# mkkellogg/GaussianSplats3D

Measured on NVIDIA H100. Metric: frames_per_sec, higher is better.
Workload: dtype int32 sort keys / f32 raster

## Files before the change

### gaussiansplats3d_b200/csrc/common.cuh

```cuda
#pragma once
#include <cuda_runtime.h>
#include <stdint.h>
#include <stdio.h>

extern thread_local char g_gs_err[512];

#include <vector>
#include <string.h>
#include <stdlib.h>

namespace gs {

__device__ __forceinline__ void pdl_enter() {
    asm volatile("griddepcontrol.launch_dependents;" ::: "memory");
    asm volatile("griddepcontrol.wait;" ::: "memory");
}
inline bool pdl_enabled() {
    static int on = -1;
    if (on < 0) { const char *v = getenv("GS_PDL"); on = (v && v[0] == '0') ? 0 : 1; }
    return on != 0;
}
template <typename... KArgs, typename... Args>
static inline void gs_launch(void (*kernel)(KArgs...), dim3 grid, dim3 block, size_t smem, cudaStream_t st, Args... args) {
    cudaLaunchConfig_t cfg{};
    cfg.gridDim = grid; cfg.blockDim = block; cfg.dynamicSmemBytes = smem; cfg.stream = st;
    cudaLaunchAttribute attr[1];
    attr[0].id = cudaLaunchAttributeProgrammaticStreamSerialization;
    attr[0].val.programmaticStreamSerializationAllowed = pdl_enabled() ? 1 : 0;
    cfg.attrs = attr; cfg.numAttrs = 1;
    (void)cudaLaunchKernelEx(&cfg, kernel, KArgs(args)...);
}

struct Profiler {
    bool on = false;
    std::vector<cudaEvent_t> ev;
    std::vector<const char *> names;
    size_t used = 0;
    void begin(cudaStream_t st) { used = 0; names.clear(); mark("<begin>", st); }
    void mark(const char *name, cudaStream_t st) {
        if (!on) return;
        if (used == ev.size()) { cudaEvent_t e; cudaEventCreate(&e); ev.push_back(e); }
        cudaEventRecord(ev[used++], st);
        names.push_back(name);
    }
    void release() { for (auto e : ev) cudaEventDestroy(e); ev.clear(); used = 0; }
};

#define GS_MAX_SCENES_DEV 32

constexpr int kRadixBits = 8;
constexpr int kRadix = 1 << kRadixBits;

__device__ __forceinline__ int4 ld_nc_v4(const void *p) {
    int4 r;
    asm volatile("ld.global.nc.L1::no_allocate.v4.s32 {%0,%1,%2,%3}, [%4];" : "=r"(r.x), "=r"(r.y), "=r"(r.z), "=r"(r.w) : "l"(p));
    return r;
}
__device__ __forceinline__ uint32_t ld_nc_u32(const void *p) {
    uint32_t r;
    asm volatile("ld.global.nc.L1::no_allocate.u32 %0, [%1];" : "=r"(r) : "l"(p));
    return r;
}
__device__ __forceinline__ uint32_t ld_volatile_u32(const uint32_t *p) {
    uint32_t r;
    asm volatile("ld.volatile.global.u32 %0, [%1];" : "=r"(r) : "l"(p) : "memory");
    return r;
}
__device__ __forceinline__ uint32_t ld_acquire_u32(const uint32_t *p) {
    uint32_t r;
    asm volatile("ld.acquire.gpu.global.u32 %0, [%1];" : "=r"(r) : "l"(p) : "memory");
    return r;
}
__device__ __forceinline__ void st_release_u32(uint32_t *p, uint32_t v) {
    asm volatile("st.release.gpu.global.u32 [%0], %1;" ::"l"(p), "r"(v) : "memory");
}
__device__ __forceinline__ uint32_t lanemask_lt() {
    uint32_t m;
    asm("mov.u32 %0, %%lanemask_lt;" : "=r"(m));
    return m;
}
__device__ __forceinline__ int warp_min(int v) {
#pragma unroll
    for (int o = 16; o > 0; o >>= 1) v = min(v, __shfl_xor_sync(0xffffffffu, v, o));
    return v;
}
__device__ __forceinline__ int warp_max(int v) {
#pragma unroll
    for (int o = 16; o > 0; o >>= 1) v = max(v, __shfl_xor_sync(0xffffffffu, v, o));
    return v;
}
__device__ __forceinline__ uint32_t warp_inclusive_scan(uint32_t v) {
    const int lane = threadIdx.x & 31;
#pragma unroll
    for (int o = 1; o < 32; o <<= 1) {
        uint32_t t = __shfl_up_sync(0xffffffffu, v, o);
        if (lane >= o) v += t;
    }
    return v;
}

template <int THREADS>
__device__ __forceinline__ uint32_t block_exclusive_scan(uint32_t v, uint32_t *smem_warp , uint32_t &total) {
    const int lane = threadIdx.x & 31, warp = threadIdx.x >> 5;
    constexpr int NW = THREADS / 32;
    const uint32_t inc = warp_inclusive_scan(v);
    if (lane == 31) smem_warp[warp] = inc;
    __syncthreads();
    if (warp == 0) {
        uint32_t w = lane < NW ? smem_warp[lane] : 0u;
        uint32_t wi = warp_inclusive_scan(w);
        smem_warp[lane] = wi - w;
        if (lane == 31) smem_warp[32] = wi;
    }
// ... 18 lines not shown
```

### gaussiansplats3d_b200/csrc/engine.cu

```cuda
#include "../../include/gsplat_b200.h"
#include "common.cuh"
#include "sort_kernels.cuh"
#include "raster_kernels.cuh"
#include "shard_kernels.cuh"
#include "ksplat_transform.h"
#include "ksplat_kernels.cuh"
#include "file_kernels.cuh"
#include "cull_kernels.cuh"

#include <algorithm>
#include <cmath>
#include <cstdarg>
#include <cstdlib>
#include <cstring>
#include <new>
#include <vector>

using namespace gs;

thread_local char g_gs_err[512] = "";
#define g_err g_gs_err
static int fail(int code, const char *fmt, ...) {
    va_list ap;
    va_start(ap, fmt);
    vsnprintf(g_err, sizeof(g_err), fmt, ap);
    va_end(ap);
    return code;
}
#define CU(call)                                                                                                  \
    do {                                                                                                          \
        cudaError_t _e = (call);                                                                                  \
        if (_e != cudaSuccess) return fail(GS_ERR_CUDA, "%s -> %s (%s:%d)", #call, cudaGetErrorString(_e), __FILE__, __LINE__); \
    } while (0)

extern "C" int gs_abi_version(void) { return GS_ABI_VERSION; }
extern "C" const char *gs_last_error_message(void) { return g_err; }
extern "C" const char *gs_status_string(int s) {
    switch (s) {
        case GS_OK: return "ok";
        case GS_ERR_BAD_ARG: return "bad argument";
        case GS_ERR_NO_DEVICE: return "no CUDA device";
        case GS_ERR_CUDA: return "CUDA error";
        case GS_ERR_DEGENERATE: return "all distances equal";
        case GS_ERR_BUCKET_RANGE: return "bucket index out of range";
        case GS_ERR_NOT_READY: return "not ready";
        case GS_ERR_CAPACITY: return "capacity exceeded";
        default: return "unknown";
    }
}
extern "C" int gs_device_count(void) {
    int n = 0;
    if (cudaGetDeviceCount(&n) != cudaSuccess) { cudaGetLastError(); return 0; }
    return n;
}

template <typename T> struct DevBuf {
    T *p = nullptr;
    size_t n = 0;
    int ensure(size_t count) {
        if (count <= n) return GS_OK;
        if (p) cudaFree(p);
        p = nullptr; n = 0;
        cudaError_t e = cudaMalloc((void **)&p, std::max<size_t>(count, 1) * sizeof(T));
        if (e != cudaSuccess) return fail(GS_ERR_CUDA, "cudaMalloc(%zu bytes) -> %s", count * sizeof(T), cudaGetErrorString(e));
        n = count;
        return GS_OK;
    }
    void release() { if (p) cudaFree(p); p = nullptr; n = 0; }
};
template <typename T> struct PinBuf {
    T *p = nullptr;
    size_t n = 0;
    int ensure(size_t count) {
        if (count <= n) return GS_OK;
        if (p) cudaFreeHost(p);
        p = nullptr; n = 0;
        cudaError_t e = cudaHostAlloc((void **)&p, std::max<size_t>(count, 1) * sizeof(T), cudaHostAllocDefault);
        if (e != cudaSuccess) return fail(GS_ERR_CUDA, "cudaHostAlloc(%zu bytes) -> %s", count * sizeof(T), cudaGetErrorString(e));
        n = count;
        return GS_OK;
    }
    void release() { if (p) cudaFreeHost(p); p = nullptr; n = 0; }
};

enum { EV_SORT0, EV_DEPTH, EV_BUCKET, EV_SORT1, EV_R0, EV_PROJECT, EV_BIN, EV_R1, EV_H2D0, EV_H2D1, EV_D2H0, EV_D2H1, EV_COUNT };

constexpr size_t kPipeSlotWords = 4 + (sizeof(RasterControl) + 3) / 4 + 12;
struct gs_engine {
    gs_config cfg{};
    cudaStream_t stream = nullptr;
    cudaEvent_t ev[EV_COUNT]{};
    int sm_count = 132;
    size_t l2_bytes = 50u << 20;
    int key_bits = 16;

    DevBuf<int4> centers;
    DevBuf<uint32_t> scene_idx;
    DevBuf<uint32_t> indexes;
    DevBuf<uint32_t> precomputed;
    DevBuf<int32_t> dist;
    DevBuf<uint32_t> keys[2];
    DevBuf<uint32_t> vals[2];
    DevBuf<uint32_t> sorted;
    DevBuf<float> transforms;
    DevBuf<SortControl> ctl;
    DevBuf<DepthParams> depthp;
    DevBuf<uint32_t> tile_hist;
    DevBuf<uint32_t> freq;
    DevBuf<int32_t> dist_rows_i;
    DevBuf<float> dist_rows_f;
    DevBuf<uint32_t> sub_idx;
    DevBuf<int32_t> sub_dist;
    uint32_t uploaded_splats = 0;
    uint32_t last_render_count = 0;
    bool have_sorted = false;
    bool ctl_dirty = true;

    PinBuf<uint32_t> h_indexes, h_sorted;
    PinBuf<uint32_t> h_ctl;
    PinBuf<unsigned char> h_frame;

    RasterState rs;

    gs_timings tm{};
    Profiler prof;
    cudaGraphExec_t graph_exec = nullptr;
    cudaStream_t stream2 = nullptr;
    cudaEvent_t ev_fork = nullptr, ev_join = nullptr;
    unsigned long long graph_key[8] = {0};
    bool graph_enabled = true;
    bool last_frame_was_graph = false;
    bool no_subset = false;
    uint32_t graph_launches = 0;
    bool have_prof_begin = false;
    bool pending_async = false;
    gs_render_params pending_rp{};
    DevBuf<uint32_t> flush;
    struct Tree {
        DevBuf<double> center, nmin, nmax;
        DevBuf<uint32_t> offsets, indexes, start;
        DevBuf<unsigned long long> key, total;
        uint32_t count = 0, splats = 0;
    } tree;
    cudaStream_t copy_stream = nullptr;
    static constexpr int kPipeRing = 4, kPipeMaxInflight = 3;
    cudaEvent_t ev_frame_done[kPipeRing] = {nullptr}, ev_copy_done[kPipeRing] = {nullptr};
    cudaStream_t param_stream = nullptr;
    cudaEvent_t ev_params[2] = {nullptr, nullptr};
    bool param_side = false;
    bool graph_snapshot[2] = {false, false};
    DevBuf<uint32_t> status_dev;
    cudaGraphExec_t graph_exec_alt = nullptr;
    unsigned long long graph_key_alt[8] = {0};
    PinBuf<uint32_t> h_pipe;
    uint64_t pipe_begun = 0, pipe_ended = 0;
    uint32_t pipe_inflight() const { return (uint32_t)(pipe_begun - pipe_ended); }

    struct Shard {
        DevBuf<unsigned char> block;
        DevBuf<uint32_t> total, ahead, block_total, delta, local_sorted;
        ShardPeers peers{};
        uint32_t *root_out = nullptr;
        void *opened[kMaxShardRanks + 1] = {nullptr};
        uint32_t world = 0, seq = 0;
        uint32_t pending_render_count = 0;
        bool attached = false, pending = false;
        bool pending_unsplit = false;
    } shard;
};

static int check_engine(gs_engine *e) {
    if (!e) return fail(GS_ERR_BAD_ARG, "null engine");
    cudaError_t ce = cudaSetDevice(e->cfg.device);
    if (ce != cudaSuccess) return fail(GS_ERR_CUDA, "cudaSetDevice(%d) -> %s", e->cfg.device, cudaGetErrorString(ce));
    return GS_OK;
}

extern "C" void gs_destroy(gs_engine *e);
#define CUE(call)                                                                                                 \
    do {                                                                                                          \
        cudaError_t _e = (call);                                                                                  \
        if (_e != cudaSuccess) {                                                                                  \
            gs_destroy(e);                                                                                        \
            return fail(GS_ERR_CUDA, "%s -> %s (%s:%d)", #call, cudaGetErrorString(_e), __FILE__, __LINE__);      \
        }                                                                                                         \
    } while (0)
extern "C" int gs_create(const gs_config *cfg, gs_engine **out) {
    if (!cfg || !out) return fail(GS_ERR_BAD_ARG, "gs_create: null argument");
    *out = nullptr;
    gs_config c{};
    memcpy(&c, cfg, std::min<size_t>(cfg->struct_size ? cfg->struct_size : sizeof(gs_config), sizeof(gs_config)));
    if (c.distance_map_range == 0) c.distance_map_range = 1u << 16;
    if (c.distance_map_range < 2 || c.distance_map_range > (1u << 24)) return fail(GS_ERR_BAD_ARG, "distance_map_range %u outside [2, 2^24]", c.distance_map_range);
    if (c.world_size == 0) { c.world_size = 1; c.rank = 0; }
    if (c.rank >= c.world_size) return fail(GS_ERR_BAD_ARG, "rank %u >= world_size %u", c.rank, c.world_size);
    int ndev = gs_device_count();
    if (ndev <= 0) return fail(GS_ERR_NO_DEVICE, "no CUDA device visible: libgsplat_b200 has no CPU path");
    if (c.device < 0 || c.device >= ndev) return fail(GS_ERR_BAD_ARG, "device %d not in [0,%d)", c.device, ndev);
    CU(cudaSetDevice(c.device));
    gs_engine *e = new (std::nothrow) gs_engine();
    if (!e) return fail(GS_ERR_BAD_ARG, "out of host memory");
    e->cfg = c;
    cudaDeviceProp prop{};
    CUE(cudaGetDeviceProperties(&prop, c.device));
    e->sm_count = prop.multiProcessorCount;
    if (prop.l2CacheSize > 0) e->l2_bytes = (size_t)prop.l2CacheSize;
    CUE(cudaStreamCreateWithFlags(&e->stream, cudaStreamNonBlocking));
    CUE(cudaStreamCreateWithFlags(&e->stream2, cudaStreamNonBlocking));
    CUE(cudaEventCreateWithFlags(&e->ev_fork, cudaEventDisableTiming));
    CUE(cudaEventCreateWithFlags(&e->ev_join, cudaEventDisableTiming));
    for (int i = 0; i < EV_COUNT; ++i) CUE(cudaEventCreate(&e->ev[i]));
    int kb = 0;
    while ((1u << kb) < c.distance_map_range) ++kb;
    e->key_bits = kb;
    int rc = GS_OK;
    const size_t n = std::max<uint32_t>(c.max_splat_count, 1);
    if ((rc = e->centers.ensure(n)) || (rc = e->indexes.ensure(n)) || (rc = e->dist.ensure(n)) || (rc = e->sorted.ensure(n)) ||
        (rc = e->vals[0].ensure(n)) || (rc = e->vals[1].ensure(n)) || (rc = e->keys[0].ensure(n)) || (rc = e->keys[1].ensure(n)) ||
        (rc = e->ctl.ensure(1)) || (rc = e->depthp.ensure(2)) || (rc = e->transforms.ensure(16 * GS_MAX_SCENES)) || (rc = e->h_ctl.ensure(sizeof(SortControl) / 4 + 64 + sizeof(RasterControl) / 4 + sizeof(ShardHeader) / 4))) {
        gs_destroy(e);
        return rc;
    }
    if (c.dynamic_mode && (rc = e->scene_idx.ensure(n))) { gs_destroy(e); return rc; }
    if (e->scene_idx.p) CUE(cudaMemsetAsync(e->scene_idx.p, 0, e->scene_idx.n * 4, e->stream));
    {
        std::vector<float> id(16 * GS_MAX_SCENES, 0.f);
        for (int s = 0; s < GS_MAX_SCENES; ++s) id[16 * s] = id[16 * s + 5] = id[16 * s + 10] = id[16 * s + 15] = 1.f;
        CUE(cudaMemcpy(e->transforms.p, id.data(), id.size() * 4, cudaMemcpyHostToDevice));
    }
    CUE(cudaMemset(e->ctl.p, 0, sizeof(SortControl)));
    rc = raster_init(e->rs, c, e->sm_count);
    if (rc) { gs_destroy(e); return fail(rc, "raster_init failed: %s", g_err); }
    if ((rc = e->status_dev.ensure(2 * kPipeSlotWords))) { gs_destroy(e); return rc; }
    CUE(cudaMemset(e->status_dev.p, 0, 2 * kPipeSlotWords * 4));
    e->rs.snap_base = e->status_dev.p;
    e->rs.snap_stride = (uint32_t)kPipeSlotWords;
    e->rs.snap_sort_ctl = reinterpret_cast<const uint32_t *>(e->ctl.p);
    CUE(cudaStreamSynchronize(e->stream));
    *out = e;
    return GS_OK;
}

#undef CUE

extern "C" void gs_destroy(gs_engine *e) {
    if (!e) return;
    cudaSetDevice(e->cfg.device);
    if (e->stream) cudaStreamSynchronize(e->stream);
    e->centers.release(); e->scene_idx.release(); e->indexes.release(); e->precomputed.release(); e->dist.release();
    e->keys[0].release(); e->keys[1].release(); e->vals[0].release(); e->vals[1].release(); e->sorted.release();
    e->transforms.release(); e->ctl.release(); e->depthp.release(); e->tile_hist.release(); e->freq.release(); e->dist_rows_i.release(); e->dist_rows_f.release(); e->sub_idx.release(); e->sub_dist.release();
    e->h_indexes.release(); e->h_sorted.release(); e->h_ctl.release(); e->h_frame.release(); e->h_pipe.release();
    e->tree.center.release(); e->tree.nmin.release(); e->tree.nmax.release(); e->tree.offsets.release(); e->tree.indexes.release(); e->tree.start.release(); e->tree.key.release(); e->tree.total.release(); e->flush.release(); e->prof.release();
    e->shard.block.release(); e->shard.total.release(); e->shard.ahead.release(); e->shard.block_total.release(); e->shard.delta.release(); e->shard.local_sorted.release();
    for (void *m : e->shard.opened) if (m) cudaIpcCloseMemHandle(m);
    if (e->rs.peer_attached) { if (e->rs.peer_frame) cudaIpcCloseMemHandle(e->rs.peer_frame); if (e->rs.peer_sync) cudaIpcCloseMemHandle(e->rs.peer_sync); }
    raster_release(e->rs);
    for (int i = 0; i < EV_COUNT; ++i) if (e->ev[i]) cudaEventDestroy(e->ev[i]);
    if (e->stream) cudaStreamDestroy(e->stream);
    if (e->stream2) cudaStreamDestroy(e->stream2);
    if (e->copy_stream) cudaStreamDestroy(e->copy_stream);
    for (int i = 0; i < gs_engine::kPipeRing; ++i) { if (e->ev_frame_done[i]) cudaEventDestroy(e->ev_frame_done[i]); if (e->ev_copy_done[i]) cudaEventDestroy(e->ev_copy_done[i]); }
    for (int i = 0; i < 2; ++i) if (e->ev_params[i]) cudaEventDestroy(e->ev_params[i]);
    if (e->param_stream) cudaStreamDestroy(e->param_stream);
    e->status_dev.release();
    if (e->graph_exec) cudaGraphExecDestroy(e->graph_exec);
    if (e->graph_exec_alt) cudaGraphExecDestroy(e->graph_exec_alt);
    if (e->ev_fork) cudaEventDestroy(e->ev_fork);
    if (e->ev_join) cudaEventDestroy(e->ev_join);
    delete e;
}

extern "C" int gs_upload_centers(gs_engine *e, const void *centers, const uint32_t *sceneIndexes, uint32_t from, uint32_t count) {
    int rc = check_engine(e);
    if (rc) return rc;
    if (!centers && count) return fail(GS_ERR_BAD_ARG, "gs_upload_centers: null centers");
    if ((uint64_t)from + count > e->cfg.max_splat_count) return fail(GS_ERR_CAPACITY, "centres [%u,%u) exceed max_splat_count %u", from, from + count, e->cfg.max_splat_count);
    if (count) CU(cudaMemcpyAsync(e->centers.p + from, centers, (size_t)count * 16, cudaMemcpyHostToDevice, e->stream));
    if (e->cfg.dynamic_mode && sceneIndexes && count)
        CU(cudaMemcpyAsync(e->scene_idx.p + from, sceneIndexes, (size_t)count * 4, cudaMemcpyHostToDevice, e->stream));
    CU(cudaStreamSynchronize(e->stream));
    e->uploaded_splats = from + count;
    return GS_OK;
}

template <int MODE>
static void launch_depth(bool identity, int blocks, cudaStream_t st, const uint32_t *idx, const void *centers, const void *pre,
                         const uint32_t *scene, const float *tr, const DepthParams *P, uint32_t s0, uint32_t rc, int32_t *dist, SortControl *ctl) {
    if (identity) gs_launch(k_depth<MODE, true>, blocks, kDepthThreads, 0, st, idx, centers, pre, scene, tr, P, s0, rc, dist, ctl);
    else gs_launch(k_depth<MODE, false>, blocks, kDepthThreads, 0, st, idx, centers, pre, scene, tr, P, s0, rc, dist, ctl);
}

static int enqueue_depth(gs_engine *e, const uint32_t *d_indexes, const float *mvp, bool use_pre, uint32_t lo, uint32_t hi, bool capturing) {
    cudaStream_t st = e->stream;
    const uint32_t n = hi - lo;
    DepthParams P{};
    memcpy(P.mvp, mvp, 64);
    P.irow[0] = (int32_t)((double)mvp[2] * 1000.0);
    P.irow[1] = (int32_t)((double)mvp[6] * 1000.0);
    P.irow[2] = (int32_t)((double)mvp[10] * 1000.0);
    P.irow[3] = 1;
    P.frow[0] = mvp[2]; P.frow[1] = mvp[6]; P.frow[2] = mvp[10]; P.frow[3] = 0.f;
    if (!capturing) CU(cudaMemcpyAsync(e->depthp.p + e->rs.frame_parity, &P, sizeof(P), cudaMemcpyHostToDevice, st));
    const bool integer = e->cfg.integer_based_sort, dyn = e->cfg.dynamic_mode;
    const int mode = use_pre ? (integer ? kIntPrecomputed : kFloatPrecomputed)
                             : (integer ? (dyn ? kIntDynamic : kIntStatic) : (dyn ? kFloatDynamic : kFloatStatic));
    const int dblocks = (int)std::max<uint64_t>(1, std::min<uint64_t>(((uint64_t)n + kDepthThreads * kDepthItems - 1) / (kDepthThreads * kDepthItems), (uint64_t)e->sm_count * 8));
    const bool identity = (d_indexes == nullptr);
    const void *pre = e->precomputed.p;
    switch (mode) {
        case kIntStatic: launch_depth<kIntStatic>(identity, dblocks, st, d_indexes, e->centers.p, pre, e->scene_idx.p, e->transforms.p, e->depthp.p + e->rs.frame_parity, lo, hi, e->dist.p, e->ctl.p); break;
        case kIntDynamic: launch_depth<kIntDynamic>(identity, dblocks, st, d_indexes, e->centers.p, pre, e->scene_idx.p, e->transforms.p, e->depthp.p + e->rs.frame_parity, lo, hi, e->dist.p, e->ctl.p); break;
        case kIntPrecomputed: launch_depth<kIntPrecomputed>(identity, dblocks, st, d_indexes, e->centers.p, pre, e->scene_idx.p, e->transforms.p, e->depthp.p + e->rs.frame_parity, lo, hi, e->dist.p, e->ctl.p); break;
        case kFloatStatic: launch_depth<kFloatStatic>(identity, dblocks, st, d_indexes, e->centers.p, pre, e->scene_idx.p, e->transforms.p, e->depthp.p + e->rs.frame_parity, lo, hi, e->dist.p, e->ctl.p); break;
        case kFloatDynamic: launch_depth<kFloatDynamic>(identity, dblocks, st, d_indexes, e->centers.p, pre, e->scene_idx.p, e->transforms.p, e->depthp.p + e->rs.frame_parity, lo, hi, e->dist.p, e->ctl.p); break;
        default: launch_depth<kFloatPrecomputed>(identity, dblocks, st, d_indexes, e->centers.p, pre, e->scene_idx.p, e->transforms.p, e->depthp.p + e->rs.frame_parity, lo, hi, e->dist.p, e->ctl.p); break;
    }
    return GS_OK;
}

static int sort_on_device(gs_engine *e, const uint32_t *d_indexes, const float *mvp, uint32_t sort_count, uint32_t render_count,
                          bool use_pre, bool write_buckets, bool capturing = false, bool subset = false, cudaEvent_t wait_for_rects = nullptr) {
    if (sort_count > render_count) return fail(GS_ERR_BAD_ARG, "sortCount %u > renderCount %u", sort_count, render_count);
    if (render_count > e->cfg.max_splat_count) return fail(GS_ERR_CAPACITY, "renderCount %u > max_splat_count %u", render_count, e->cfg.max_splat_count);
    cudaStream_t st = e->stream;
    const uint32_t s0 = render_count - sort_count, n = sort_count;
    const PassPlan pl = make_plan_bits(e->key_bits);
    uint32_t launches = 0;
    uint32_t stride = 0;
    int rc = e->tile_hist.ensure(radix_tile_hist_words(std::max(n, 1u), pl.npasses, &stride));
    if (rc) return rc;
    if (!capturing) CU(cudaEventRecord(e->ev[EV_SORT0], st));
    if (!e->have_prof_begin) e->prof.begin(st);
    if (e->ctl_dirty && !capturing) {
        gs_launch(k_sort_init, 1, 256, 0, st, e->ctl.p);
        ++launches;
    }
    if (!capturing) e->ctl_dirty = true;
    if (s0 > 0) { gs_launch(k_copy_head, std::min<uint32_t>((s0 + 255) / 256, e->sm_count * 8), 256, 0, st, d_indexes, e->sorted.p, s0); ++launches; e->prof.mark("k_copy_head", st); }
    if (n > 0) {
        if ((rc = enqueue_depth(e, d_indexes, mvp, use_pre, s0, render_count, capturing))) return rc;
        const bool identity = (d_indexes == nullptr);
        ++launches;
        e->prof.mark("k_depth", st);
        if (!capturing) CU(cudaEventRecord(e->ev[EV_DEPTH], st));
        const uint32_t tiles = (n + kRadixTile - 1) / kRadixTile;
        const uint32_t R = e->cfg.distance_map_range;
        const uint32_t *vsrc = identity ? nullptr : d_indexes + s0;
        int vmode = identity ? kValIotaReversed : kValArrayReversed;
        int32_t *dist_sorted = e->dist.p + s0;
        const unsigned long long *n_dev = nullptr;
        if (subset) {
            if (wait_for_rects) CU(cudaStreamWaitEvent(st, wait_for_rects, 0));
            int rcs = raster_subset(e->rs, e->cfg, d_indexes, render_count, e->dist.p, e->sub_idx.p, e->sub_dist.p, st, e->prof, launches);
            if (rcs) return rcs;
            vsrc = e->sub_idx.p; vmode = kValArrayReversed;
            dist_sorted = e->sub_dist.p;
            n_dev = &e->rs.rctl.p->subset_count;
        }
        static const RadixNames names = {{"k_radix_hist[depth,0]", "k_radix_hist[depth,1]", "k_radix_hist[depth,2]", "k_radix_hist[depth,3]"},
                                         {"k_radix_scan[depth,0]", "k_radix_scan[depth,1]", "k_radix_scan[depth,2]", "k_radix_scan[depth,3]"},
                                         {"k_radix_scatter[depth,0]", "k_radix_scatter[depth,1]", "k_radix_scatter[depth,2]", "k_radix_scatter[depth,3]"}};
        if (e->key_bits <= 16) {
            gs_launch(k_bucket<uint16_t>, tiles, kRadixThreads, 0, st, dist_sorted, (uint16_t *)e->keys[0].p, n, n_dev, R, pl, write_buckets ? 1 : 0, e->ctl.p, e->tile_hist.p, stride);
            ++launches;
            e->prof.mark("k_bucket", st);
            if (!capturing) CU(cudaEventRecord(e->ev[EV_BUCKET], st));
            radix_sort_pairs<uint16_t, uint32_t>((uint16_t *)e->keys[0].p, (uint16_t *)e->keys[1].p, vsrc, render_count - 1u, vmode, e->vals[0].p, e->vals[1].p,
                                       e->sorted.p + s0, n, n_dev, (unsigned long long)n, pl, e->ctl.p, e->tile_hist.p, stride, true, nullptr, st, launches, &e->prof, names, true);
        } else {
            gs_launch(k_bucket<uint32_t>, tiles, kRadixThreads, 0, st, dist_sorted, e->keys[0].p, n, n_dev, R, pl, write_buckets ? 1 : 0, e->ctl.p, e->tile_hist.p, stride);
            ++launches;
            e->prof.mark("k_bucket", st);
            if (!capturing) CU(cudaEventRecord(e->ev[EV_BUCKET], st));
            radix_sort_pairs<uint32_t, uint32_t>(e->keys[0].p, e->keys[1].p, vsrc, render_count - 1u, vmode, e->vals[0].p, e->vals[1].p, e->sorted.p + s0, n,
                                       n_dev, (unsigned long long)n, pl, e->ctl.p, e->tile_hist.p, stride, true, nullptr, st, launches, &e->prof, names, true);
        }
    } else if (!capturing) {
        CU(cudaEventRecord(e->ev[EV_DEPTH], st));
        CU(cudaEventRecord(e->ev[EV_BUCKET], st));
    }
    if (!capturing) CU(cudaEventRecord(e->ev[EV_SORT1], st));
    CU(cudaGetLastError());
    e->tm.kernel_launches = launches;
    e->last_render_count = render_count;
    e->have_sorted = true;
    if (!capturing) e->ctl_dirty = false;
    return GS_OK;
}

static int finish_sort(gs_engine *e, float *sort_time_ms) {
    CU(cudaMemcpyAsync(e->h_ctl.p, e->ctl.p, 12, cudaMemcpyDeviceToHost, e->stream));
    CU(cudaStreamSynchronize(e->stream));
    float ms = 0.f;
    if (e->last_frame_was_graph) {
        e->tm.depth_ms = e->tm.bucket_ms = e->tm.scatter_ms = 0.f;
        cudaEventElapsedTime(&ms, e->ev[EV_SORT0], e->ev[EV_R1]);
    } else {
        cudaEventElapsedTime(&e->tm.depth_ms, e->ev[EV_SORT0], e->ev[EV_DEPTH]);
        cudaEventElapsedTime(&e->tm.bucket_ms, e->ev[EV_DEPTH], e->ev[EV_BUCKET]);
        cudaEventElapsedTime(&e->tm.scatter_ms, e->ev[EV_BUCKET], e->ev[EV_SORT1]);
        cudaEventElapsedTime(&ms, e->ev[EV_SORT0], e->ev[EV_SORT1]);
    }
    e->tm.sort_total_ms = ms;
    if (sort_time_ms) *sort_time_ms = ms;
    const uint32_t err = e->h_ctl.p[2];
    if (err & kErrBucketRange) return fail(GS_ERR_BUCKET_RANGE, "a bucket index fell outside [0,%u): distances overflow the int32/f32 range map", e->cfg.distance_map_range);
    return GS_OK;
}

static int stage_sort_inputs(gs_engine *e, const gs_sort_params *p, const uint32_t **d_indexes) {
    cudaStream_t st = e->stream;
    *d_indexes = nullptr;
    CU(cudaEventRecord(e->ev[EV_H2D0], st));
    if (p->indexes_to_sort_dev) *d_indexes = p->indexes_to_sort_dev;
    else if (p->indexes_to_sort) {
        CU(cudaMemcpyAsync(e->indexes.p, p->indexes_to_sort, (size_t)p->render_count * 4, cudaMemcpyHostToDevice, st));
        *d_indexes = e->indexes.p;
    }
    if (e->cfg.dynamic_mode && p->transforms) CU(cudaMemcpyAsync(e->transforms.p, p->transforms, 16 * GS_MAX_SCENES * 4, cudaMemcpyHostToDevice, st));
    if (p->use_precomputed_distances) {
        if (!p->precomputed_distances) return fail(GS_ERR_BAD_ARG, "use_precomputed_distances without precomputed_distances");
        int rc = e->precomputed.ensure(e->cfg.max_splat_count);
        if (rc) return rc;
        CU(cudaMemcpyAsync(e->precomputed.p, p->precomputed_distances, (size_t)e->uploaded_splats * 4, cudaMemcpyHostToDevice, st));
    }
    CU(cudaEventRecord(e->ev[EV_H2D1], st));
    return GS_OK;
}

extern "C" int gs_sort(gs_engine *e, const gs_sort_params *p, uint32_t *sorted_out, float *sort_time_ms) {
    int rc = check_engine(e);
    if (rc) return rc;
    if (!p) return fail(GS_ERR_BAD_ARG, "gs_sort: null params");
    gs_sort_params q = *p;
    q.render_count = std::min(q.render_count, e->uploaded_splats);
    q.sort_count = std::min(q.sort_count, e->uploaded_splats);
    if (q.sort_count > q.render_count) return fail(GS_ERR_BAD_ARG, "sortCount %u > renderCount %u", q.sort_count, q.render_count);
    const uint32_t *d_idx = nullptr;
    e->last_frame_was_graph = false;
    if ((rc = stage_sort_inputs(e, &q, &d_idx))) return rc;
    if ((rc = sort_on_device(e, d_idx, q.model_view_proj, q.sort_count, q.render_count, q.use_precomputed_distances != 0, false))) return rc;
    CU(cudaEventRecord(e->ev[EV_D2H0], e->stream));
    if (sorted_out && q.render_count) CU(cudaMemcpyAsync(sorted_out, e->sorted.p, (size_t)q.render_count * 4, cudaMemcpyDeviceToHost, e->stream));
    CU(cudaEventRecord(e->ev[EV_D2H1], e->stream));
    rc = finish_sort(e, sort_time_ms);
    cudaEventElapsedTime(&e->tm.h2d_ms, e->ev[EV_H2D0], e->ev[EV_H2D1]);
    cudaEventElapsedTime(&e->tm.d2h_ms, e->ev[EV_D2H0], e->ev[EV_D2H1]);
    return rc;
// ... 1177 lines not shown
```

### gaussiansplats3d_b200/csrc/sort_kernels.cuh

```cuda
#pragma once
#include "common.cuh"

namespace gs {

enum DepthMode : int {
    kIntStatic = 0, kIntDynamic = 1, kIntPrecomputed = 2, kFloatStatic = 3, kFloatDynamic = 4, kFloatPrecomputed = 5
};

struct DepthParams {
    int32_t irow[4];
    float frow[4];
    float mvp[16];
};

__global__ void k_sort_init(SortControl *ctl) {
    pdl_enter();
    const uint32_t tid = threadIdx.x;
    if (tid == 0) {
        ctl->dmin = 2147483640;
        ctl->dmax = -2147483640;
        ctl->error = 0;
    }
    uint32_t *h = &ctl->hist[0][0];
    for (uint32_t i = tid; i < 4 * kRadix; i += blockDim.x) h[i] = 0;
}

__device__ __forceinline__ void scene_row(const float *mvp, const float *t, float out[4]) {
#pragma unroll
    for (int c = 0; c < 4; ++c) {
        float acc = __fmul_rn(mvp[2], t[4 * c + 0]);
        acc = __fadd_rn(acc, __fmul_rn(mvp[6], t[4 * c + 1]));
        acc = __fadd_rn(acc, __fmul_rn(mvp[10], t[4 * c + 2]));
        acc = __fadd_rn(acc, __fmul_rn(mvp[14], t[4 * c + 3]));
        out[c] = acc;
    }
}
__device__ __forceinline__ int32_t trunc_scaled(float f, double scale) { return __double2int_rz((double)f * scale); }

template <int MODE>
__device__ __forceinline__ int32_t splat_distance(uint32_t g, const void *__restrict__ centers, const void *__restrict__ pre,
                                                  const uint32_t *__restrict__ scene_idx, const DepthParams &P,
                                                  const int32_t (*s_irow)[4], const float (*s_frow)[4]) {
    if (MODE == kIntPrecomputed) return (int32_t)ld_nc_u32((const uint32_t *)pre + g);
    if (MODE == kFloatPrecomputed) return trunc_scaled(__uint_as_float(ld_nc_u32((const uint32_t *)pre + g)), 4096.0);
    const int4 c = ld_nc_v4((const int4 *)centers + g);
    if (MODE == kIntStatic) {
        return (int32_t)((uint32_t)P.irow[0] * (uint32_t)c.x + (uint32_t)P.irow[1] * (uint32_t)c.y + (uint32_t)P.irow[2] * (uint32_t)c.z);
    } else if (MODE == kIntDynamic) {
        const int32_t *r = s_irow[ld_nc_u32(scene_idx + g) & (GS_MAX_SCENES_DEV - 1)];
        return (int32_t)((uint32_t)r[0] * (uint32_t)c.x + (uint32_t)r[1] * (uint32_t)c.y + (uint32_t)r[2] * (uint32_t)c.z +
                         (uint32_t)r[3] * (uint32_t)c.w);
    } else if (MODE == kFloatStatic) {
        float acc = __fmul_rn(P.frow[0], __int_as_float(c.x));
        acc = __fadd_rn(acc, __fmul_rn(P.frow[1], __int_as_float(c.y)));
        acc = __fadd_rn(acc, __fmul_rn(P.frow[2], __int_as_float(c.z)));
        return trunc_scaled(acc, 4096.0);
    } else {
        const float *r = s_frow[ld_nc_u32(scene_idx + g) & (GS_MAX_SCENES_DEV - 1)];
        float acc = __fmul_rn(r[0], __int_as_float(c.x));
        acc = __fadd_rn(acc, __fmul_rn(r[1], __int_as_float(c.y)));
        acc = __fadd_rn(acc, __fmul_rn(r[2], __int_as_float(c.z)));
        acc = __fadd_rn(acc, __fmul_rn(r[3], __int_as_float(c.w)));
        return trunc_scaled(acc, 4096.0);
    }
}

constexpr int kDepthThreads = 256;
constexpr int kDepthItems = 4;

template <int MODE, bool IDENTITY>
__global__ void __launch_bounds__(kDepthThreads)
k_depth(const uint32_t *__restrict__ indexes, const void *__restrict__ centers, const void *__restrict__ pre,
        const uint32_t *__restrict__ scene_idx, const float *__restrict__ transforms, const DepthParams *__restrict__ Pp, uint32_t s0,
        uint32_t rc, int32_t *__restrict__ dist, SortControl *ctl) {
    pdl_enter();
    DepthParams P;
#pragma unroll
    for (int i = 0; i < 4; ++i) { P.irow[i] = __ldg(&Pp->irow[i]); P.frow[i] = __ldg(&Pp->frow[i]); }
    if (MODE == kIntDynamic || MODE == kFloatDynamic) {
#pragma unroll
        for (int i = 0; i < 16; ++i) P.mvp[i] = __ldg(&Pp->mvp[i]);
    }
    __shared__ int32_t s_irow[GS_MAX_SCENES_DEV][4];
// ... 229 lines not shown
        for (int w = 0; w < kRadixWarps; ++w) {
            const uint32_t c = s_whist[w][tid];
            s_whist[w][tid] = run;
            run += c;
        }
        s_tile_count[tid] = run;
    }
    __syncthreads();
    {
        uint32_t total;
        const uint32_t c = tid < kRadix ? s_tile_count[tid] : 0u;
        const uint32_t ex = block_exclusive_scan<kRadixThreads>(c, s_scan, total);
        if (tid < kRadix) { s_tile_start[tid] = ex; s_gbase[tid] = my_offset - ex; }
    }
    __syncthreads();
#pragma unroll
    for (int k = 0; k < kRadixItems; ++k) {
        const uint32_t d = (key[k] >> shift) & dmask;
        rank[k] = (FULL || key[k] != 0xffffffffu) ? (s_tile_start[d] + s_whist[warp][d] + rank[k]) : 0xffffffffu;
    }
    __syncthreads();
#pragma unroll
    for (int k = 0; k < kRadixItems; ++k) {
        const uint32_t e = run_base + (uint32_t)k * 32;
        if (FULL || rank[k] != 0xffffffffu) {
            ValT v;
            if (VALMODE == kValArray) v = __ldg(vals_in + e);
            else if (VALMODE == kValArrayReversed) v = __ldg(vals_in + (n - 1u - e));
            else v = (ValT)(iota_top - e);
            s_vals[rank[k]] = v;
            s_keys[rank[k]] = (KeyT)key[k];
        }
    }
    __syncthreads();
    const uint32_t valid = FULL ? (uint32_t)kRadixTile : (n - tile_base);
#pragma unroll
    for (int k = 0; k < kRadixItems; ++k) {
        const uint32_t q = (uint32_t)k * kRadixThreads + tid;
        if (FULL || q < valid) {
            const KeyT kk = s_keys[q];
            const uint32_t d = ((uint32_t)kk >> shift) & dmask;
            const uint32_t dst = s_gbase[d] + q;
            vals_out[dst] = s_vals[q];
            if (WRITE_KEYS) keys_out[dst] = kk;
            if (RANGES) {
                if (q == 0 || s_keys[q - 1] != kk) atomicMin(&ranges[(uint32_t)kk].x, dst);
                if (q + 1 == valid || s_keys[q + 1] != kk) atomicMax(&ranges[(uint32_t)kk].y, dst + 1u);
            }
        }
    }
}

template <typename KeyT, typename ValT, int VALMODE, bool WRITE_KEYS, bool RANGES>
__global__ void __launch_bounds__(kRadixThreads, 2)
k_radix_scatter(const KeyT *__restrict__ keys_in, const ValT *__restrict__ vals_in, uint32_t iota_top,
                KeyT *__restrict__ keys_out, ValT *__restrict__ vals_out, uint32_t n_host,
                const unsigned long long *__restrict__ n_dev, unsigned long long n_cap, int shift, int bits,
                const uint32_t *__restrict__ tile_offsets, uint32_t stride, uint2 *ranges, uint32_t *clear_hist, SortControl *reset_ctl) {
    pdl_enter();
    const uint32_t n = n_dev ? (uint32_t)min(*n_dev, n_cap) : n_host;
    const uint32_t tile = blockIdx.x;
    if (tile == 0) {
        if (clear_hist && threadIdx.x < kRadix) clear_hist[threadIdx.x] = 0;
        if (reset_ctl && threadIdx.x == 0) { reset_ctl->dmin = 2147483640; reset_ctl->dmax = -2147483640; }
    }
    const uint64_t tile_base = (uint64_t)tile * kRadixTile;
    if (tile_base >= n) return;
    __shared__ __align__(16) unsigned char s_raw[kRadixTile * (sizeof(KeyT) + sizeof(ValT)) > kRadixWarps * (kRadix + 1) * 4
                                                     ? kRadixTile * (sizeof(KeyT) + sizeof(ValT))
                                                     : kRadixWarps * (kRadix + 1) * 4];
    __shared__ uint32_t s_tile_count[kRadix];
    __shared__ uint32_t s_tile_start[kRadix];
    __shared__ uint32_t s_gbase[kRadix];
    __shared__ uint32_t s_scan[40];
    const uint32_t dmask = (1u << bits) - 1u;
    if (tile_base + kRadixTile <= n)
        radix_scatter_tile<KeyT, ValT, VALMODE, WRITE_KEYS, RANGES, true>(keys_in, vals_in, iota_top, keys_out, vals_out, n, tile, shift, dmask, tile_offsets, stride,
                                                                          ranges, s_raw, s_tile_count, s_tile_start, s_gbase, s_scan);
    else
        radix_scatter_tile<KeyT, ValT, VALMODE, WRITE_KEYS, RANGES, false>(keys_in, vals_in, iota_top, keys_out, vals_out, n, tile, shift, dmask, tile_offsets, stride,
                                                                           ranges, s_raw, s_tile_count, s_tile_start, s_gbase, s_scan);
}

__global__ void k_copy_head(const uint32_t *__restrict__ indexes, uint32_t *__restrict__ out, uint32_t s0) {
    pdl_enter();
    for (uint64_t i = (uint64_t)blockIdx.x * blockDim.x + threadIdx.x; i < s0; i += (uint64_t)gridDim.x * blockDim.x)
        out[i] = indexes ? indexes[i] : (uint32_t)i;
}

__global__ void k_bucket_counts(const int32_t *__restrict__ buckets, uint32_t s0, uint32_t rc, uint32_t *counts) {
    for (uint64_t i = (uint64_t)s0 + (uint64_t)blockIdx.x * blockDim.x + threadIdx.x; i < rc; i += (uint64_t)gridDim.x * blockDim.x)
        atomicAdd(&counts[buckets[i]], 1u);
}
__global__ void __launch_bounds__(1024) k_exclusive_scan_single_block(uint32_t *data, uint32_t n) {
    __shared__ uint32_t s_scan[40];
    __shared__ uint32_t s_carry;
    if (threadIdx.x == 0) s_carry = 0;
    __syncthreads();
    for (uint32_t base = 0; base < n; base += 1024) {
        const uint32_t i = base + threadIdx.x;
        const uint32_t v = i < n ? data[i] : 0u;
        uint32_t total;
        const uint32_t ex = block_exclusive_scan<1024>(v, s_scan, total);
        const uint32_t carry = s_carry;
        if (i < n) data[i] = ex + carry;
        __syncthreads();
        if (threadIdx.x == 0) s_carry = carry + total;
        __syncthreads();
    }
}

template <bool INTEGER, bool DYNAMIC>
__global__ void k_distances_splat_order(const void *__restrict__ centers, const uint32_t *__restrict__ scene_idx,
                                        const int32_t *__restrict__ irows , const float *__restrict__ frows,
                                        uint32_t count, void *__restrict__ out) {
    for (uint64_t i = (uint64_t)blockIdx.x * blockDim.x + threadIdx.x; i < count; i += (uint64_t)gridDim.x * blockDim.x) {
        const int4 c = ld_nc_v4((const int4 *)centers + i);
        const uint32_t sc = DYNAMIC ? (scene_idx[i] & (GS_MAX_SCENES_DEV - 1)) : 0u;
        if (INTEGER) {
            const int32_t *r = irows + 4 * sc;
            uint32_t d = (uint32_t)c.x * (uint32_t)r[0] + (uint32_t)c.y * (uint32_t)r[1] + (uint32_t)c.z * (uint32_t)r[2];
            if (DYNAMIC) d += (uint32_t)r[3] * (uint32_t)c.w;
            ((int32_t *)out)[i] = (int32_t)d;
        } else {
            const float *r = frows + 4 * sc;
            float acc = __fmul_rn(__int_as_float(c.x), r[0]);
            acc = __fadd_rn(acc, __fmul_rn(__int_as_float(c.y), r[1]));
            acc = __fadd_rn(acc, __fmul_rn(__int_as_float(c.z), r[2]));
            if (DYNAMIC) acc = __fadd_rn(acc, r[3]);
            ((float *)out)[i] = acc;
        }
    }
}


static inline PassPlan make_plan_bits(int key_bits) {
    PassPlan pl{};
    int np = (key_bits + kRadixBits - 1) / kRadixBits;
    if (np < 1) np = 1;
    pl.npasses = np;
    int done = 0;
    for (int p = 0; p < np; ++p) {
        const int left = key_bits - done, b = (left + (np - p) - 1) / (np - p);
        pl.shift[p] = done;
        pl.bits[p] = b < 1 ? 1 : b;
        done += b;
    }
    return pl;
}

template <typename KeyT, typename ValT>
static void launch_radix_scatter(uint32_t grid, bool first, bool write_keys, bool want_ranges, int valmode, const KeyT *kin, const ValT *vin,
                                 uint32_t iota_top, KeyT *kout, ValT *vout, uint32_t n, const unsigned long long *n_dev, unsigned long long n_cap,
                                 int shift, int bits, const uint32_t *tile_offsets, uint32_t stride, uint2 *ranges, uint32_t *clear_hist, SortControl *reset_ctl,
                                 cudaStream_t st) {
#define GS_PASS(VM, WK, RG) gs_launch(k_radix_scatter<KeyT, ValT, VM, WK, RG>, grid, kRadixThreads, 0, st, kin, vin, iota_top, kout, vout, n, n_dev, n_cap, shift, bits, tile_offsets, stride, ranges, clear_hist, reset_ctl)
    if (!first) valmode = kValArray;
    if (want_ranges && !write_keys) { GS_PASS(kValArray, false, true); }
    else if (want_ranges) {
        if (valmode == kValArray) GS_PASS(kValArray, true, true);
        else if (valmode == kValArrayReversed) GS_PASS(kValArrayReversed, true, true);
        else GS_PASS(kValIotaReversed, true, true);
    }
    else if (valmode == kValArray) { if (!write_keys) GS_PASS(kValArray, false, false); else GS_PASS(kValArray, true, false); }
    else if (valmode == kValArrayReversed) { if (!write_keys) GS_PASS(kValArrayReversed, false, false); else GS_PASS(kValArrayReversed, true, false); }
    else { if (!write_keys) GS_PASS(kValIotaReversed, false, false); else GS_PASS(kValIotaReversed, true, false); }
// ... 49 lines not shown
```

Baseline: 3301.

## Fuse depth and bucket passes into one cooperative kernel with grid sync

Adds a cooperative kernel that computes splat depths into shared memory, reduces the global min/max, runs a grid-wide sync, and then buckets the depths, writes 16-bit keys and builds the first radix histogram. It replaces the separate k_depth and k_bucket launches when keys fit in 16 bits. This removes one launch and the global round trip of the depth array between the two passes. In exchange, grid size is capped by co-residency (at most one tile per CTA), and the kernel pays for a grid barrier and a high-priority cooperative launch.

```diff
diff --git a/gaussiansplats3d_b200/csrc/common.cuh b/gaussiansplats3d_b200/csrc/common.cuh
--- a/gaussiansplats3d_b200/csrc/common.cuh
+++ b/gaussiansplats3d_b200/csrc/common.cuh
@@ -29,6 +29,20 @@
     attr[0].val.programmaticStreamSerializationAllowed = pdl_enabled() ? 1 : 0;
     cfg.attrs = attr; cfg.numAttrs = 1;
     (void)cudaLaunchKernelEx(&cfg, kernel, KArgs(args)...);
+}
+template <typename... KArgs, typename... Args>
+static inline cudaError_t gs_launch_coop(void (*kernel)(KArgs...), dim3 grid, dim3 block, size_t smem, cudaStream_t st, int priority, Args... args) {
+    cudaLaunchConfig_t cfg{};
+    cfg.gridDim = grid; cfg.blockDim = block; cfg.dynamicSmemBytes = smem; cfg.stream = st;
+    cudaLaunchAttribute attr[3];
+    attr[0].id = cudaLaunchAttributeCooperative;
+    attr[0].val.cooperative = 1;
+    attr[1].id = cudaLaunchAttributePriority;
+    attr[1].val.priority = priority;
+    attr[2].id = cudaLaunchAttributeProgrammaticStreamSerialization;
+    attr[2].val.programmaticStreamSerializationAllowed = pdl_enabled() ? 1 : 0;
+    cfg.attrs = attr; cfg.numAttrs = 3;
+    return cudaLaunchKernelEx(&cfg, kernel, KArgs(args)...);
 }
 
 struct Profiler {
diff --git a/gaussiansplats3d_b200/csrc/engine.cu b/gaussiansplats3d_b200/csrc/engine.cu
--- a/gaussiansplats3d_b200/csrc/engine.cu
+++ b/gaussiansplats3d_b200/csrc/engine.cu
@@ -93,6 +93,8 @@
     int sm_count = 132;
     size_t l2_bytes = 50u << 20;
     int key_bits = 16;
+    uint32_t coop_grid = 0;
+    int coop_priority = 0;
 
     DevBuf<int4> centers;
     DevBuf<uint32_t> scene_idx;
@@ -174,6 +176,33 @@
     cudaError_t ce = cudaSetDevice(e->cfg.device);
     if (ce != cudaSuccess) return fail(GS_ERR_CUDA, "cudaSetDevice(%d) -> %s", e->cfg.device, cudaGetErrorString(ce));
     return GS_OK;
+}
+
+template <typename F> static int coop_occupancy(F f) {
+    const size_t smem = kDepthBucketTiles * kDepthBucketTileSmem;
+    int b = 0;
+    if (cudaFuncSetAttribute(f, cudaFuncAttributeMaxDynamicSharedMemorySize, (int)smem) != cudaSuccess ||
+        cudaOccupancyMaxActiveBlocksPerMultiprocessor(&b, f, kDepthBucketThreads, smem) != cudaSuccess)
+        b = 0;
+    return b;
+}
+template <int MODE> static int coop_occupancy_mode() { return std::min(coop_occupancy(k_depth_bucket<MODE, true>), coop_occupancy(k_depth_bucket<MODE, false>)); }
+static void coop_prepare(gs_engine *e) {
+    e->coop_grid = 0;
+    int coop = 0;
+    if (e->key_bits > 16 || cudaDeviceGetAttribute(&coop, cudaDevAttrCooperativeLaunch, e->cfg.device) != cudaSuccess || !coop) {
+        (void)cudaGetLastError();
+        return;
+    }
+    const bool integer = e->cfg.integer_based_sort, dyn = e->cfg.dynamic_mode;
+    const int own = integer ? (dyn ? coop_occupancy_mode<kIntDynamic>() : coop_occupancy_mode<kIntStatic>())
+                            : (dyn ? coop_occupancy_mode<kFloatDynamic>() : coop_occupancy_mode<kFloatStatic>());
+    const int pre = integer ? coop_occupancy_mode<kIntPrecomputed>() : coop_occupancy_mode<kFloatPrecomputed>();
+    int least = 0, greatest = 0;
+    if (cudaDeviceGetStreamPriorityRange(&least, &greatest) != cudaSuccess) greatest = 0;
+    (void)cudaGetLastError();
+    e->coop_grid = (uint32_t)std::max(0, std::min(own, pre)) * (uint32_t)e->sm_count;
+    e->coop_priority = greatest;
 }
 
 extern "C" void gs_destroy(gs_engine *e);
@@ -213,6 +242,7 @@
     int kb = 0;
     while ((1u << kb) < c.distance_map_range) ++kb;
     e->key_bits = kb;
+    coop_prepare(e);
     int rc = GS_OK;
     const size_t n = std::max<uint32_t>(c.max_splat_count, 1);
     if ((rc = e->centers.ensure(n)) || (rc = e->indexes.ensure(n)) || (rc = e->dist.ensure(n)) || (rc = e->sorted.ensure(n)) ||
@@ -291,9 +321,7 @@
     else gs_launch(k_depth<MODE, false>, blocks, kDepthThreads, 0, st, idx, centers, pre, scene, tr, P, s0, rc, dist, ctl);
 }
 
-static int enqueue_depth(gs_engine *e, const uint32_t *d_indexes, const float *mvp, bool use_pre, uint32_t lo, uint32_t hi, bool capturing) {
-    cudaStream_t st = e->stream;
-    const uint32_t n = hi - lo;
+static int stage_depth_params(gs_engine *e, const float *mvp, bool use_pre, bool capturing, int *mode) {
     DepthParams P{};
     memcpy(P.mvp, mvp, 64);
     P.irow[0] = (int32_t)((double)mvp[2] * 1000.0);
@@ -301,10 +329,19 @@
     P.irow[2] = (int32_t)((double)mvp[10] * 1000.0);
     P.irow[3] = 1;
     P.frow[0] = mvp[2]; P.frow[1] = mvp[6]; P.frow[2] = mvp[10]; P.frow[3] = 0.f;
-    if (!capturing) CU(cudaMemcpyAsync(e->depthp.p + e->rs.frame_parity, &P, sizeof(P), cudaMemcpyHostToDevice, st));
+    if (!capturing) CU(cudaMemcpyAsync(e->depthp.p + e->rs.frame_parity, &P, sizeof(P), cudaMemcpyHostToDevice, e->stream));
     const bool integer = e->cfg.integer_based_sort, dyn = e->cfg.dynamic_mode;
-    const int mode = use_pre ? (integer ? kIntPrecomputed : kFloatPrecomputed)
-                             : (integer ? (dyn ? kIntDynamic : kIntStatic) : (dyn ? kFloatDynamic : kFloatStatic));
+    *mode = use_pre ? (integer ? kIntPrecomputed : kFloatPrecomputed)
+                    : (integer ? (dyn ? kIntDynamic : kIntStatic) : (dyn ? kFloatDynamic : kFloatStatic));
+    return GS_OK;
+}
+
+static int enqueue_depth(gs_engine *e, const uint32_t *d_indexes, const float *mvp, bool use_pre, uint32_t lo, uint32_t hi, bool capturing) {
+    cudaStream_t st = e->stream;
+    const uint32_t n = hi - lo;
+    int mode = 0;
+    int rc = stage_depth_params(e, mvp, use_pre, capturing, &mode);
+    if (rc) return rc;
     const int dblocks = (int)std::max<uint64_t>(1, std::min<uint64_t>(((uint64_t)n + kDepthThreads * kDepthItems - 1) / (kDepthThreads * kDepthItems), (uint64_t)e->sm_count * 8));
     const bool identity = (d_indexes == nullptr);
     const void *pre = e->precomputed.p;
@@ -319,6 +356,52 @@
     return GS_OK;
 }
 
+template <int MODE>
+static cudaError_t launch_depth_bucket(bool identity, uint32_t grid, uint32_t tpc, int prio, cudaStream_t st, const uint32_t *idx, const void *centers,
+                                       const void *pre, const uint32_t *scene, const float *tr, const DepthParams *P, uint32_t s0, uint32_t n, uint32_t R,
+                                       PassPlan pl, int wb, int32_t *dist, uint16_t *keys, uint32_t *tile_hist, uint32_t stride, SortControl *ctl) {
+    const size_t smem = tpc * kDepthBucketTileSmem;
+    if (identity) return gs_launch_coop(k_depth_bucket<MODE, true>, grid, kDepthBucketThreads, smem, st, prio, idx, centers, pre, scene, tr, P, s0, n, tpc, R, pl, wb, dist, keys, tile_hist, stride, ctl);
+    return gs_launch_coop(k_depth_bucket<MODE, false>, grid, kDepthBucketThreads, smem, st, prio, idx, centers, pre, scene, tr, P, s0, n, tpc, R, pl, wb, dist, keys, tile_hist, stride, ctl);
+}
+
+static int enqueue_depth_bucket(gs_engine *e, const uint32_t *d_indexes, const float *mvp, bool use_pre, uint32_t s0, uint32_t n, bool write_buckets,
+                                bool capturing, uint32_t stride, bool *launched) {
+    *launched = false;
+    const uint32_t tiles = (n + kRadixTile - 1) / kRadixTile;
+    if (!e->coop_grid || e->key_bits > 16 || !tiles) return GS_OK;
+    const uint32_t tpc = (tiles + e->coop_grid - 1) / e->coop_grid;
+    if (tpc > (uint32_t)kDepthBucketTiles) return GS_OK;
+    const uint32_t grid = (tiles + tpc - 1) / tpc;
+    int mode = 0;
+    int rc = stage_depth_params(e, mvp, use_pre, capturing, &mode);
+    if (rc) return rc;
+    const bool identity = (d_indexes == nullptr);
+    const PassPlan pl = make_plan_bits(e->key_bits);
+    const uint32_t R = e->cfg.distance_map_range;
+    const int wb = write_buckets ? 1 : 0, prio = e->coop_priority;
+    cudaStream_t st = e->stream;
+    const void *pre = e->precomputed.p;
+    const DepthParams *P = e->depthp.p + e->rs.frame_parity;
+    uint16_t *keys = (uint16_t *)e->keys[0].p;
+    cudaError_t ce;
+    switch (mode) {
+        case kIntStatic: ce = launch_depth_bucket<kIntStatic>(identity, grid, tpc, prio, st, d_indexes, e->centers.p, pre, e->scene_idx.p, e->transforms.p, P, s0, n, R, pl, wb, e->dist.p, keys, e->tile_hist.p, stride, e->ctl.p); break;
+        case kIntDynamic: ce = launch_depth_bucket<kIntDynamic>(identity, grid, tpc, prio, st, d_indexes, e->centers.p, pre, e->scene_idx.p, e->transforms.p, P, s0, n, R, pl, wb, e->dist.p, keys, e->tile_hist.p, stride, e->ctl.p); break;
+        case kIntPrecomputed: ce = launch_depth_bucket<kIntPrecomputed>(identity, grid, tpc, prio, st, d_indexes, e->centers.p, pre, e->scene_idx.p, e->transforms.p, P, s0, n, R, pl, wb, e->dist.p, keys, e->tile_hist.p, stride, e->ctl.p); break;
+        case kFloatStatic: ce = launch_depth_bucket<kFloatStatic>(identity, grid, tpc, prio, st, d_indexes, e->centers.p, pre, e->scene_idx.p, e->transforms.p, P, s0, n, R, pl, wb, e->dist.p, keys, e->tile_hist.p, stride, e->ctl.p); break;
+        case kFloatDynamic: ce = launch_depth_bucket<kFloatDynamic>(identity, grid, tpc, prio, st, d_indexes, e->centers.p, pre, e->scene_idx.p, e->transforms.p, P, s0, n, R, pl, wb, e->dist.p, keys, e->tile_hist.p, stride, e->ctl.p); break;
+        default: ce = launch_depth_bucket<kFloatPrecomputed>(identity, grid, tpc, prio, st, d_indexes, e->centers.p, pre, e->scene_idx.p, e->transforms.p, P, s0, n, R, pl, wb, e->dist.p, keys, e->tile_hist.p, stride, e->ctl.p); break;
+    }
+    if (ce != cudaSuccess) {
+        (void)cudaGetLastError();
+        if (capturing) return fail(GS_ERR_CUDA, "cooperative depth + bucket pass (%u CTAs) refused inside a graph capture: %s", grid, cudaGetErrorString(ce));
+        return GS_OK;
+    }
+    *launched = true;
+    return GS_OK;
+}
+
 static int sort_on_device(gs_engine *e, const uint32_t *d_indexes, const float *mvp, uint32_t sort_count, uint32_t render_count,
                           bool use_pre, bool write_buckets, bool capturing = false, bool subset = false, cudaEvent_t wait_for_rects = nullptr) {
     if (sort_count > render_count) return fail(GS_ERR_BAD_ARG, "sortCount %u > renderCount %u", sort_count, render_count);
@@ -339,11 +422,19 @@
     if (!capturing) e->ctl_dirty = true;
     if (s0 > 0) { gs_launch(k_copy_head, std::min<uint32_t>((s0 + 255) / 256, e->sm_count * 8), 256, 0, st, d_indexes, e->sorted.p, s0); ++launches; e->prof.mark("k_copy_head", st); }
     if (n > 0) {
-        if ((rc = enqueue_depth(e, d_indexes, mvp, use_pre, s0, render_count, capturing))) return rc;
         const bool identity = (d_indexes == nullptr);
-        ++launches;
-        e->prof.mark("k_depth", st);
-        if (!capturing) CU(cudaEventRecord(e->ev[EV_DEPTH], st));
+        bool fused = false;
+        if (!subset && (rc = enqueue_depth_bucket(e, d_indexes, mvp, use_pre, s0, n, write_buckets, capturing, stride, &fused))) return rc;
+        if (fused) {
+            ++launches;
+            e->prof.mark("k_depth_bucket[depth]", st);
+            if (!capturing) CU(cudaEventRecord(e->ev[EV_DEPTH], st));
+        } else {
+            if ((rc = enqueue_depth(e, d_indexes, mvp, use_pre, s0, render_count, capturing))) return rc;
+            ++launches;
+            e->prof.mark("k_depth", st);
+            if (!capturing) CU(cudaEventRecord(e->ev[EV_DEPTH], st));
+        }
         const uint32_t tiles = (n + kRadixTile - 1) / kRadixTile;
         const uint32_t R = e->cfg.distance_map_range;
         const uint32_t *vsrc = identity ? nullptr : d_indexes + s0;
@@ -362,9 +453,11 @@
                                          {"k_radix_scan[depth,0]", "k_radix_scan[depth,1]", "k_radix_scan[depth,2]", "k_radix_scan[depth,3]"},
                                          {"k_radix_scatter[depth,0]", "k_radix_scatter[depth,1]", "k_radix_scatter[depth,2]", "k_radix_scatter[depth,3]"}};
         if (e->key_bits <= 16) {
-            gs_launch(k_bucket<uint16_t>, tiles, kRadixThreads, 0, st, dist_sorted, (uint16_t *)e->keys[0].p, n, n_dev, R, pl, write_buckets ? 1 : 0, e->ctl.p, e->tile_hist.p, stride);
-            ++launches;
-            e->prof.mark("k_bucket", st);
+            if (!fused) {
+                gs_launch(k_bucket<uint16_t>, tiles, kRadixThreads, 0, st, dist_sorted, (uint16_t *)e->keys[0].p, n, n_dev, R, pl, write_buckets ? 1 : 0, e->ctl.p, e->tile_hist.p, stride);
+                ++launches;
+                e->prof.mark("k_bucket", st);
+            }
             if (!capturing) CU(cudaEventRecord(e->ev[EV_BUCKET], st));
             radix_sort_pairs<uint16_t, uint32_t>((uint16_t *)e->keys[0].p, (uint16_t *)e->keys[1].p, vsrc, render_count - 1u, vmode, e->vals[0].p, e->vals[1].p,
                                        e->sorted.p + s0, n, n_dev, (unsigned long long)n, pl, e->ctl.p, e->tile_hist.p, stride, true, nullptr, st, launches, &e->prof, names, true);
diff --git a/gaussiansplats3d_b200/csrc/sort_kernels.cuh b/gaussiansplats3d_b200/csrc/sort_kernels.cuh
--- a/gaussiansplats3d_b200/csrc/sort_kernels.cuh
+++ b/gaussiansplats3d_b200/csrc/sort_kernels.cuh
@@ -1,4 +1,5 @@
 #pragma once
+#include <cooperative_groups.h>
 #include "common.cuh"
 
 namespace gs {
@@ -394,6 +395,115 @@
                                                                            ranges, s_raw, s_tile_count, s_tile_start, s_gbase, s_scan);
 }
 
+constexpr int kDepthBucketThreads = 512;
+constexpr int kDepthBucketTiles = 1;
+constexpr size_t kDepthBucketTileSmem = (size_t)kRadixTile * 4;
+
+template <int MODE, bool IDENTITY>
+__global__ void __launch_bounds__(kDepthBucketThreads)
+k_depth_bucket(const uint32_t *__restrict__ indexes, const void *__restrict__ centers, const void *__restrict__ pre,
+               const uint32_t *__restrict__ scene_idx, const float *__restrict__ transforms, const DepthParams *__restrict__ Pp, uint32_t s0,
+               uint32_t n, uint32_t tiles_per_cta, uint32_t R, PassPlan plan, int write_buckets, int32_t *__restrict__ dist,
+               uint16_t *__restrict__ keys, uint32_t *__restrict__ tile_hist, uint32_t stride, SortControl *ctl) {
+    asm volatile("griddepcontrol.wait;" ::: "memory");
+    extern __shared__ __align__(16) int32_t s_dist[];
+    __shared__ uint32_t s_hist[kRadix];
+    __shared__ int32_t s_irow[GS_MAX_SCENES_DEV][4];
+    __shared__ float s_frow[GS_MAX_SCENES_DEV][4];
+    __shared__ int s_min[kDepthBucketThreads / 32], s_max[kDepthBucketThreads / 32];
+    const uint32_t tid = threadIdx.x, t0 = blockIdx.x * tiles_per_cta;
+    const uint32_t lo = (uint32_t)min((uint64_t)n, (uint64_t)t0 * kRadixTile);
+    const uint32_t hi = (uint32_t)min((uint64_t)n, (uint64_t)lo + (uint64_t)tiles_per_cta * kRadixTile);
+    const uint32_t cnt = hi - lo, itop = s0 + n - 1u;
+
+    DepthParams P;
+#pragma unroll
+    for (int i = 0; i < 4; ++i) { P.irow[i] = __ldg(&Pp->irow[i]); P.frow[i] = __ldg(&Pp->frow[i]); }
+    if (MODE == kIntDynamic || MODE == kFloatDynamic) {
+#pragma unroll
+        for (int i = 0; i < 16; ++i) P.mvp[i] = __ldg(&Pp->mvp[i]);
+        if (tid < GS_MAX_SCENES_DEV) {
+            float row[4];
+            scene_row(P.mvp, transforms + 16 * tid, row);
+#pragma unroll
+            for (int k = 0; k < 4; ++k) {
+                s_frow[tid][k] = row[k];
+                s_irow[tid][k] = trunc_scaled(row[k], 1000.0);
+            }
+        }
+        __syncthreads();
+    }
+    if (blockIdx.x == 0 && tid == 0) ctl->error = 0;
+    int32_t lmin = 2147483640, lmax = -2147483640;
+    for (uint32_t base = 0; base < cnt; base += kDepthBucketThreads * kDepthItems) {
+        int32_t d[kDepthItems];
+#pragma unroll
+        for (int k = 0; k < kDepthItems; ++k) {
+            const uint32_t q = base + (uint32_t)k * kDepthBucketThreads + tid;
+            if (q < cnt) {
+                const uint32_t i = itop - (lo + q);
+                d[k] = splat_distance<MODE>(IDENTITY ? i : ld_nc_u32(indexes + i), centers, pre, scene_idx, P, s_irow, s_frow);
+            }
+        }
+#pragma unroll
+        for (int k = 0; k < kDepthItems; ++k) {
+            const uint32_t q = base + (uint32_t)k * kDepthBucketThreads + tid;
+            if (q < cnt) {
+                s_dist[q] = d[k];
+                if (!write_buckets) dist[itop - (lo + q)] = d[k];
+                lmin = min(lmin, d[k]);
+                lmax = max(lmax, d[k]);
+            }
+        }
+    }
+    lmin = warp_min(lmin);
+    lmax = warp_max(lmax);
+    if ((tid & 31) == 0) { s_min[tid >> 5] = lmin; s_max[tid >> 5] = lmax; }
+    __syncthreads();
+    if (tid < 32) {
+        lmin = warp_min(tid < kDepthBucketThreads / 32 ? s_min[tid] : 2147483640);
+        lmax = warp_max(tid < kDepthBucketThreads / 32 ? s_max[tid] : -2147483640);
+        if (tid == 0 && cnt) { atomicMin(&ctl->dmin, lmin); atomicMax(&ctl->dmax, lmax); }
+    }
+    cooperative_groups::this_grid().sync();
+    asm volatile("griddepcontrol.launch_dependents;" ::: "memory");
+
+    const int32_t dmin = __ldcg(&ctl->dmin), dmax = __ldcg(&ctl->dmax);
+    const float span = __fsub_rn(__int2float_rn(dmax), __int2float_rn(dmin));
+    const float range_map = __fdiv_rn(__uint2float_rn(R - 1u), span);
+    const bool degenerate = (dmax == dmin);
+    const uint32_t mask0 = (1u << plan.bits[0]) - 1u;
+    uint32_t err = 0;
+    for (uint32_t t = 0; t < tiles_per_cta && t * (uint32_t)kRadixTile < cnt; ++t) {
+        if (tid < kRadix) s_hist[tid] = 0;
+        __syncthreads();
+#pragma unroll
+        for (int k = 0; k < kRadixItems; ++k) {
+            const uint32_t q = t * (uint32_t)kRadixTile + (uint32_t)k * kDepthBucketThreads + tid;
+            if (q < cnt) {
+                const int32_t rel = (int32_t)((uint32_t)s_dist[q] - (uint32_t)dmin);
+                int32_t b = __float2int_rz(__fmul_rn(__int2float_rn(rel), range_map));
+                if (degenerate) b = 0;
+                if (rel < 0 || b < 0) { err |= kErrBucketRange; b = 0; }
+                else if ((uint32_t)b >= R) b = (int32_t)(R - 1u);
+                if (write_buckets) dist[itop - (lo + q)] = b;
+                const uint32_t key = (R - 1u) - (uint32_t)b;
+                keys[lo + q] = (uint16_t)key;
+                atomicAdd(&s_hist[(key >> plan.shift[0]) & mask0], 1u);
+            }
+        }
+        __syncthreads();
+        if (tid < kRadix) {
+            const uint32_t v = s_hist[tid];
+            tile_hist[(size_t)tid * stride + t0 + t] = v;
+            if (v) atomicAdd(&ctl->hist[0][tid], v);
+        }
+        __syncthreads();
+    }
+    if (err) atomicOr(&ctl->error, err);
+    if (degenerate && blockIdx.x == 0 && tid == 0) atomicOr(&ctl->error, kErrDegenerate);
+}
+
 __global__ void k_copy_head(const uint32_t *__restrict__ indexes, uint32_t *__restrict__ out, uint32_t s0) {
     pdl_enter();
     for (uint64_t i = (uint64_t)blockIdx.x * blockDim.x + threadIdx.x; i < s0; i += (uint64_t)gridDim.x * blockDim.x)
```

New measurement: 3306, median of 6. No clear change (+0.2%).
